# KieDani/UpliftingTableTennis

Measured on NVIDIA B200. Metric: frames_per_sec_detect_decode, higher is better.
Workload: dtype tf32

## Files before the change

### upliftingtabletennis_b200/csrc/conv_umma.cu

```cuda
#include <cuda.h>

#include <string.h>

#include <algorithm>
#include <vector>

#include "hrnet.h"
#include "umma_prims.h"

namespace {

using namespace umma;

constexpr int BW = 128;
constexpr int THREADS = 192;
constexpr int THREADS_HF = 320;

constexpr int pow2_cols(int c) { return c <= 32 ? 32 : c <= 64 ? 64 : c <= 128 ? 128 : c <= 256 ? 256 : 512; }
constexpr int al1024(int b) { return (b + 1023) & ~1023; }

template <int KS, int S, int CIN, int COUT, int R, int STAGES, int RB, int KCO = 0, int ESZ = 2, int HF = 0>
struct Cfg {
  static constexpr int KCMAX = 128 / ESZ;
  static constexpr int KC = KCO ? KCO : (CIN < KCMAX ? CIN : KCMAX);
  static constexpr int NKC = CIN / KC;
  static constexpr int ROWB = KC * ESZ;
  static constexpr int KSTEPS = ROWB / 32;
  static constexpr int PAD = KS / 2;
  static constexpr bool FUSE = KS == 3 && S == 1 && 3 * COUT <= 256;
  static constexpr int NPY = S == 2 ? 2 : 1;
  static constexpr int NBOX = S == 2 ? 2 : 1;
  static constexpr int TW = S == 2 ? BW + 1 : (HF ? BW : BW + 2 * PAD);
  static constexpr int OUTW = HF ? BW - 2 : BW;
  static constexpr int TR = S == 2 ? R + 1 : R + 2 * PAD;
  static constexpr int BOX_BYTES = TR * TW * ROWB;
  static constexpr int BOX_AL = al1024(BOX_BYTES);
  static constexpr int STAGE_BYTES = NBOX * BOX_AL;
// ... 19 lines not shown
  static constexpr uint32_t SWZ = ROWB == 32 ? 1u : ROWB == 64 ? 3u : 7u;
  static_assert(S == 1 || KS == 3, "stride 2 is implemented for 3x3 only");
  static_assert(!HF || (KS == 3 && S == 1 && 9 * COUT <= 256 && COUT == 16 && !RB), "horizontal tap fusion: 3x3 stride 1, 16 output channels, no staged residual");
  static_assert(2 * ACC_COLS <= 512, "accumulators exceed TMEM");
  static constexpr bool PIPE = S == 1 && !RB && !HF && ACC_COLS >= 64 && (ESZ == 4 || COUT >= 64);
  static constexpr int GMAX = (ESZ == 2 && !PIPE) ? 64 : 32;
  static constexpr int GCOLS = ACC_COLS < GMAX ? ACC_COLS : GMAX;
  static_assert(ESZ == 2 || ESZ == 4, "bf16 or tf32-in-fp32 elements");
  static_assert(ACC_COLS % GCOLS == 0, "the epilogue drains whole groups of accumulator columns");
  static_assert(ROWB == 32 || ROWB == 64 || ROWB == 128, "a K-chunk is one 32/64/128-byte swizzled row");
  static_assert(COUT % 16 == 0 && COUT <= 256 && CIN % 16 == 0, "bad channel counts");
  static_assert(SMEM_BYTES <= 232448, "shared memory budget");
};

struct KMaps {
  CUtensorMap m[4];
  CUtensorMap res;
};

struct KArgs {
  const void* w;
  const float* bias;
  void* out;
  const void* res[3];
  int rsh[3];
  int nres;
  int res_tma;
  int dual;
  int n, h, w_img, cout_total;
  int relu;
  int tiles_x, tiles_y, total;
};

template <int KS, int S, int CIN, int COUT, int R, int STAGES, int RB, int KCO = 0, int ESZ = 2, int HF = 0>
__global__ void __launch_bounds__(HF ? THREADS_HF : THREADS, 1) conv_umma_kernel(const __grid_constant__ KMaps maps, const KArgs a) {
  constexpr int NTHR = HF ? THREADS_HF : THREADS;
  using C = Cfg<KS, S, CIN, COUT, R, STAGES, RB, KCO, ESZ, HF>;
  extern __shared__ uint8_t smem_raw[];
  uint8_t* smem = reinterpret_cast<uint8_t*>((reinterpret_cast<uintptr_t>(smem_raw) + 1023) & ~(uintptr_t)1023);
  uint8_t* sW = smem;
  uint8_t* sA = smem + C::W_BYTES_AL;
  uint8_t* sR = sA + STAGES * C::STAGE_BYTES;
  float* sBias = reinterpret_cast<float*>(sR + C::RES_BYTES);
  float* sXch = sBias + COUT;
  uint64_t* bars = reinterpret_cast<uint64_t*>(sXch + C::XCH_BYTES / 4);
  uint32_t* tmem_slot = reinterpret_cast<uint32_t*>(bars + 2 * STAGES + 6);
  uint8_t* sStage = reinterpret_cast<uint8_t*>((reinterpret_cast<uintptr_t>(bars) + 256 + 127) & ~(uintptr_t)127);
  const uint32_t bar_full = smem_u32(bars), bar_empty = bar_full + 8 * STAGES, bar_tfull = bar_empty + 8 * STAGES,
                 bar_tempty = bar_tfull + 16, bar_rfull = bar_tempty + 16;
  const int tid = threadIdx.x, warp = tid >> 5, lane = tid & 31;
  const int n_off = blockIdx.y * COUT;
  const bool res_tma = RB && a.res_tma;

  {
    const uint4* wsrc = reinterpret_cast<const uint4*>(a.w) + (size_t)blockIdx.y * (C::W_BYTES / 16);
    const uint32_t wbase = smem_u32(sW);
    constexpr int CPR = C::ROWB / 16;
    for (int i = tid; i < C::W_BYTES / 16; i += NTHR) {
      uint32_t addr = wbase + (i / CPR) * C::ROWB + (i % CPR) * 16;
      addr ^= ((addr >> 7) & C::SWZ) << 4;
      *reinterpret_cast<uint4*>(sW + (addr - wbase)) = __ldg(wsrc + i);
    }
    for (int i = tid; i < COUT; i += NTHR) sBias[i] = a.bias[n_off + i];
  }
  if (tid == 0) {
    for (int s = 0; s < STAGES; ++s) {
      mbar_init(bar_full + 8 * s, 1);
      mbar_init(bar_empty + 8 * s, 1);
    }
    for (int i = 0; i < 2; ++i) {
// ... 131 lines not shown
    const int q = warp & 3;
    const int m = q * 32 + lane;
    constexpr int GCOLS = C::GCOLS;
    constexpr int NSUB = GCOLS / 16;
    constexpr int RW = 4 * ESZ;
    const uint32_t lane_base = tmem + ((uint32_t)(q * 32) << 16);
    const int eg = (warp - 2) >> 2;
    if (eg == 0)
      for (int c = 0; c < 2 * C::ACC_COLS; c += 16) tmem_zero16(lane_base + c);
    tmem_wait_st();
    fence_before();
    __syncwarp();
    if (lane == 0) {
      mbar_arrive(bar_tempty);
      mbar_arrive(bar_tempty + 8);
    }
    auto add_words = [](float* f, const uint32_t* w) {
      if (ESZ == 2) {
#pragma unroll
        for (int j = 0; j < 8; ++j) {
          f[2 * j] += __uint_as_float(w[j] << 16);
          f[2 * j + 1] += __uint_as_float(w[j] & 0xffff0000u);
        }
      } else {
#pragma unroll
        for (int j = 0; j < 16; ++j) f[j] += __uint_as_float(w[j]);
      }
    };
    uint32_t tcount = 0;
    for (int tile = blockIdx.x; tile < a.total; tile += gridDim.x, ++tcount) {
      const int tx = tile % a.tiles_x, ty = (tile / a.tiles_x) % a.tiles_y, img = tile / (a.tiles_x * a.tiles_y);
      const uint32_t acc = tcount & 1, aph = (tcount >> 1) & 1;
      const int ox = HF ? tx * C::OUTW + m - 1 : tx * BW + m;
      if (res_tma) mbar_wait(bar_rfull + 8 * acc, aph);
      mbar_wait(bar_tfull + 8 * acc, aph);
      fence_after();
      if constexpr (HF != 0) {
        const uint32_t tbase = lane_base + acc * C::ACC_COLS;
        float* xme = sXch + (q * 2) * R * COUT;
#pragma unroll 1
        for (int r = eg; r < R; r += 2) {
          uint32_t e0[16], e2[16];
          tmem_ld16(tbase + (R - 1 - r) * 3 * COUT, e0);
          tmem_ld16(tbase + (R - 1 - r) * 3 * COUT + 2 * COUT, e2);
          tmem_wait_ld();
          if (lane == 31) {
#pragma unroll
            for (int j = 0; j < 16; ++j) xme[r * COUT + j] = __uint_as_float(e0[j]);
          }
          if (lane == 0) {
#pragma unroll
            for (int j = 0; j < 16; ++j) xme[R * COUT + r * COUT + j] = __uint_as_float(e2[j]);
          }
        }
        asm volatile("bar.sync 1, 256;" ::: "memory");
        const float* xprev = sXch + ((q > 0 ? q - 1 : 0) * 2) * R * COUT;
        const float* xnext = sXch + ((q < 3 ? q + 1 : 3) * 2 + 1) * R * COUT;
#pragma unroll 1
        for (int r = eg; r < R; r += 2) {
          uint32_t v0[16], v1[16], v2[16];
          const uint32_t ta = tbase + (R - 1 - r) * 3 * COUT;
          tmem_ld16(ta, v0);
          tmem_ld16(ta + COUT, v1);
          tmem_ld16(ta + 2 * COUT, v2);
          tmem_wait_ld();
          tmem_zero16(ta);
// ... 122 lines not shown
            if (!(ox < a.w_img && oy < a.h)) continue;
            float f[16];
#pragma unroll
            for (int j = 0; j < 16; ++j) f[j] = __uint_as_float(v[g & 1][sb][j]) + sBias[c0 + j];
            if (nres > 0) add_words(f, rv[g & 1][sb]);
            if (a.relu) {
#pragma unroll
              for (int j = 0; j < 16; ++j) f[j] = fmaxf(f[j], 0.f);
            }
            char* op = (char*)a.out + ((((size_t)img * a.h + oy) * a.w_img + ox) * a.cout_total + n_off + c0) * ESZ;
            if (ESZ == 2) {
              uint32_t o[8];
#pragma unroll
              for (int j = 0; j < 8; ++j) {
                __nv_bfloat162 b2 = __floats2bfloat162_rn(f[2 * j], f[2 * j + 1]);
                o[j] = *reinterpret_cast<uint32_t*>(&b2);
              }
              stg256(op, o);
            } else {
              uint32_t o[16];
#pragma unroll
              for (int j = 0; j < 16; ++j) o[j] = __float_as_uint(f[j]);
              stg256(op, o);
              stg256(op + 32, o + 8);
            }
          }
          if (g + 1 < G) {
            tmem_wait_ld();
#pragma unroll
            for (int sb = 0; sb < NSUB; ++sb) tmem_zero16(tbase + (g + 1) * GCOLS + sb * 16);
          }
        }
      } else {
#pragma unroll 1
      for (int g0 = 0; g0 < C::ACC_COLS; g0 += GCOLS) {
        uint32_t v[NSUB][16];
        const uint32_t taddr = lane_base + acc * C::ACC_COLS + g0;
#pragma unroll
        for (int sb = 0; sb < NSUB; ++sb) tmem_ld16(taddr + sb * 16, v[sb]);
        uint32_t rv[NSUB][RW], rx[NSUB][2][RW];
        const int nres = a.nres;
#pragma unroll
        for (int sb = 0; sb < NSUB; ++sb) {
          const int col = g0 + sb * 16, r = R - 1 - col / COUT, c0 = col % COUT;
          const int oy = ty * R + r;
          const bool live = ox < a.w_img && oy < a.h;
#pragma unroll
          for (int j = 0; j < RW; ++j) rv[sb][j] = 0;
          if (nres > 0) {
            if (res_tma) {
              const uint32_t row = smem_u32(sR + (acc * C::NRB + c0 / C::CB) * C::RBOX_BYTES) + (r * BW + m) * C::RROWB;
              const uint32_t swz = ((row >> 7) & C::RSWZ) << 4;
#pragma unroll
              for (int i = 0; i < RW / 4; ++i) lds128((row + (c0 % C::CB) * ESZ + 16 * i) ^ swz, &rv[sb][4 * i]);
            } else if (live) {
              const int sh = a.rsh[0];
              const char* rp = (const char*)a.res[0] +
                               ((((size_t)img * (a.h >> sh) + (oy >> sh)) * (a.w_img >> sh) + (ox >> sh)) * a.cout_total + n_off + c0) * ESZ;
#pragma unroll
              for (int i = 0; i < RW / 8; ++i) ldg256(rp + 32 * i, &rv[sb][8 * i]);
            }
#pragma unroll
            for (int rr = 1; rr < 3; ++rr) {
              if (rr < nres && live) {
                const int sh = a.rsh[rr];
                const char* rp = (const char*)a.res[rr] +
                                 ((((size_t)img * (a.h >> sh) + (oy >> sh)) * (a.w_img >> sh) + (ox >> sh)) * a.cout_total + n_off + c0) * ESZ;
#pragma unroll
                for (int i = 0; i < RW / 8; ++i) ldg256(rp + 32 * i, &rx[sb][rr - 1][8 * i]);
              }
            }
          }
        }
        tmem_wait_ld();
#pragma unroll
        for (int sb = 0; sb < NSUB; ++sb) tmem_zero16(taddr + sb * 16);
#pragma unroll
        for (int sb = 0; sb < NSUB; ++sb) {
          const int col = g0 + sb * 16, r = R - 1 - col / COUT, c0 = col % COUT;
          const int oy = ty * R + r;
          if (!(ox < a.w_img && oy < a.h)) continue;
          float f[16];
#pragma unroll
          for (int j = 0; j < 16; ++j) f[j] = __uint_as_float(v[sb][j]) + sBias[c0 + j];
          if (nres > 0) {
            add_words(f, rv[sb]);
#pragma unroll
            for (int rr = 1; rr < 3; ++rr) {
              if (rr >= nres) break;
              add_words(f, rx[sb][rr - 1]);
            }
          }
          if (a.relu) {
#pragma unroll
            for (int j = 0; j < 16; ++j) f[j] = fmaxf(f[j], 0.f);
          }
          char* op = (char*)a.out + ((((size_t)img * a.h + oy) * a.w_img + ox) * a.cout_total + n_off + c0) * ESZ;
          if (ESZ == 2) {
            uint32_t o[8];
#pragma unroll
            for (int j = 0; j < 8; ++j) {
              __nv_bfloat162 b2 = __floats2bfloat162_rn(f[2 * j], f[2 * j + 1]);
              o[j] = *reinterpret_cast<uint32_t*>(&b2);
            }
            stg256(op, o);
          } else {
            uint32_t o[16];
#pragma unroll
            for (int j = 0; j < 16; ++j) o[j] = __float_as_uint(f[j]);
            stg256(op, o);
            stg256(op + 32, o + 8);
          }
        }
      }
      }
      tmem_wait_st();
      fence_before();
      __syncwarp();
      if (lane == 0) mbar_arrive(bar_tempty + 8 * acc);
    }
  }
  fence_before();
  __syncthreads();
  if (warp == 2) tmem_dealloc(tmem, C::TMEM_COLS);
}

int cout_tile(const TtkConv& cv, int esz) { return (cv.k == 3 && cv.cout_p == 128 && cv.cin_p >= 64) ? (esz == 2 ? 64 : 32) : cv.cout_p; }
bool fused_ky(const TtkConv& cv, int esz) { return cv.k == 3 && cv.stride == 1 && 3 * cout_tile(cv, esz) <= 256; }
bool fused_h(const TtkConv& cv, int esz) { return esz == 4 && cv.k == 3 && cv.stride == 1 && cv.cin_p == 128 && cv.cout_p == 16; }
int kc_of(const TtkConv& cv, int esz) {
  if (esz == 2) {
    if (cv.k == 3 && cv.stride == 1 && cv.cin_p >= 64) return 32;
    if (cv.k == 3 && cv.stride == 2 && cv.cin_p >= 64) return 32;
    return cv.cin_p < 64 ? cv.cin_p : 64;
  }
  if (cv.k == 3 && cv.stride == 1 && cv.cin_p == 128 && cv.cout_p == 16) return 16;
  if (cv.k == 3 && cv.cin_p >= 64) return 8;
  if (cv.k == 3 && cv.stride == 2 && cv.cin_p == 32 && cv.cout_p == 128) return 8;
  if (cv.k == 3) return 16;
  return 32;
}

CUtensorMapSwizzle swizzle_for(int row_bytes) {
  return row_bytes == 32 ? CU_TENSOR_MAP_SWIZZLE_32B : row_bytes == 64 ? CU_TENSOR_MAP_SWIZZLE_64B : CU_TENSOR_MAP_SWIZZLE_128B;
}

float round_tf32(float v) {
  uint32_t u;
  memcpy(&u, &v, 4);
  u += 0xfffu + ((u >> 13) & 1u);
  u &= ~0x1fffu;
  memcpy(&v, &u, 4);
  return v;
}

template <int KS, int S, int CIN, int COUT, int R, int STAGES, int RB, int KCO = 0, int ESZ = 2, int HF = 0>
int launch(const TtkConv& cv, const ConvLaunch& a, cudaStream_t st) {
  using C = Cfg<KS, S, CIN, COUT, R, STAGES, RB, KCO, ESZ, HF>;
  if (C::KC != kc_of(cv, ESZ) || COUT != cout_tile(cv, ESZ) || (HF != 0) != fused_h(cv, ESZ)) {
    ttk_set_error("conv %s: kernel K-chunk %d / output slice %d differ from the packed weights' %d / %d", cv.name.c_str(), C::KC, COUT,
                  kc_of(cv, ESZ), cout_tile(cv, ESZ));
    return TTK_ERR_STATE;
  }
  EncodeFn encode = get_encode();
  if (!encode) {
    ttk_set_error("cuTensorMapEncodeTiled is not available from the driver");
    return TTK_ERR_CUDA;
  }
  static TtkPerDevice attr;
  if (attr.first()) {
    TTK_CUDA(cudaFuncSetAttribute(conv_umma_kernel<KS, S, CIN, COUT, R, STAGES, RB, KCO, ESZ, HF>, cudaFuncAttributeMaxDynamicSharedMemorySize,
                                  C::SMEM_BYTES));
  }
  if (S == 2 && ((a.hin & 1) || (a.win & 1))) return TTK_ERR_UNSUPPORTED;
  const CUtensorMapDataType in_type = ESZ == 2 ? CU_TENSOR_MAP_DATA_TYPE_BFLOAT16 : CU_TENSOR_MAP_DATA_TYPE_TFLOAT32;
  const CUtensorMapDataType res_type = ESZ == 2 ? CU_TENSOR_MAP_DATA_TYPE_BFLOAT16 : CU_TENSOR_MAP_DATA_TYPE_FLOAT32;
  KMaps maps;
  cuuint32_t box[4] = {(cuuint32_t)C::KC, (cuuint32_t)C::TW, (cuuint32_t)C::TR, 1};
  cuuint32_t es[4] = {1, 1, 1, 1};
  for (int i = 0; i < (S == 2 ? 4 : 1); ++i) {
    const int py = i >> 1, px = i & 1;
    cuuint64_t dims[4] = {(cuuint64_t)CIN, (cuuint64_t)(a.win / S), (cuuint64_t)(a.hin / S), (cuuint64_t)a.n};
    cuuint64_t strides[3] = {(cuuint64_t)CIN * ESZ * S, (cuuint64_t)a.win * CIN * ESZ * S, (cuuint64_t)a.hin * a.win * CIN * ESZ};
    void* base = (char*)const_cast<void*>(a.in) + ((size_t)py * a.win + px) * CIN * ESZ;
    const CUresult r = encode(&maps.m[i], in_type, 4, base, dims, strides, box, es, CU_TENSOR_MAP_INTERLEAVE_NONE, swizzle_for(C::ROWB),
                              CU_TENSOR_MAP_L2_PROMOTION_L2_256B, CU_TENSOR_MAP_FLOAT_OOB_FILL_NONE);
    if (r != CUDA_SUCCESS) {
      ttk_set_error("cuTensorMapEncodeTiled failed (%d) for conv %s", (int)r, cv.name.c_str());
      return TTK_ERR_CUDA;
    }
  }
  for (int i = (S == 2 ? 4 : 1); i < 4; ++i) maps.m[i] = maps.m[0];
  const bool res_tma = RB && a.nres > 0 && a.res_shift[0] == 0;
  maps.res = maps.m[0];
  if (res_tma) {
    cuuint64_t dims[4] = {(cuuint64_t)a.cout, (cuuint64_t)a.wout, (cuuint64_t)a.hout, (cuuint64_t)a.n};
    cuuint64_t strides[3] = {(cuuint64_t)a.cout * ESZ, (cuuint64_t)a.wout * a.cout * ESZ, (cuuint64_t)a.hout * a.wout * a.cout * ESZ};
    cuuint32_t rbox[4] = {(cuuint32_t)C::CB, (cuuint32_t)BW, (cuuint32_t)R, 1};
    const CUresult r = encode(&maps.res, res_type, 4, const_cast<void*>(a.res[0]), dims, strides, rbox, es, CU_TENSOR_MAP_INTERLEAVE_NONE,
                              swizzle_for(C::RROWB), CU_TENSOR_MAP_L2_PROMOTION_L2_256B, CU_TENSOR_MAP_FLOAT_OOB_FILL_NONE);
    if (r != CUDA_SUCCESS) {
      ttk_set_error("cuTensorMapEncodeTiled (residual) failed (%d) for conv %s", (int)r, cv.name.c_str());
      return TTK_ERR_CUDA;
    }
  }
  KArgs k;
  k.w = ESZ == 2 ? (const void*)cv.w_umma : (const void*)cv.w_umma32;
  k.bias = cv.bias;
  k.out = a.out;
  for (int i = 0; i < 3; ++i) {
    k.res[i] = a.res[i];
    k.rsh[i] = a.res_shift[i];
  }
  k.nres = a.nres;
  k.res_tma = res_tma ? 1 : 0;
  k.dual = 0;
  k.n = a.n;
  k.h = a.hout;
  k.w_img = a.wout;
  k.cout_total = a.cout;
  k.relu = a.relu;
  k.tiles_x = ttk_cdiv(a.wout, C::OUTW);
  k.tiles_y = ttk_cdiv(a.hout, R);
  k.total = k.tiles_x * k.tiles_y * a.n;
  const int nsplit = a.cout / COUT;
  int occ = std::min(232448 / (C::SMEM_BYTES + 1024), 512 / C::TMEM_COLS);
  occ = std::max(1, std::min(occ, 2));
  const int gx = std::max(1, std::min(k.total, ttk_num_sms() * occ / nsplit));
  dim3 grid(gx, nsplit);
  conv_umma_kernel<KS, S, CIN, COUT, R, STAGES, RB, KCO, ESZ, HF><<<grid, HF ? THREADS_HF : THREADS, C::SMEM_BYTES, st>>>(maps, k);
  TTK_LAUNCH_CHECK();
  return TTK_OK;
}

template <int ESZ>
int launch_dual(const void* w_dual, const float* bias_dual, const ConvLaunch& a, cudaStream_t st) {
  constexpr int R = 2, STAGES = 3, KC = 128 / ESZ, CINK = ESZ == 2 ? 128 : 96;
  using C = Cfg<1, 1, CINK, 128, R, STAGES, 0, 0, ESZ>;
  EncodeFn encode = get_encode();
  if (!encode) return TTK_ERR_UNSUPPORTED;
  static TtkPerDevice attr;
  if (attr.first()) {
    TTK_CUDA(cudaFuncSetAttribute(conv_umma_kernel<1, 1, CINK, 128, R, STAGES, 0, 0, ESZ>, cudaFuncAttributeMaxDynamicSharedMemorySize, C::SMEM_BYTES));
  }
  KMaps maps;
  cuuint32_t box[4] = {(cuuint32_t)KC, (cuuint32_t)BW, (cuuint32_t)R, 1};
  cuuint32_t es[4] = {1, 1, 1, 1};
  const void* ins[2] = {a.in, a.in2};
  const int cins[2] = {a.cin, a.cin2};
  for (int i = 0; i < 2; ++i) {
    cuuint64_t dims[4] = {(cuuint64_t)cins[i], (cuuint64_t)a.win, (cuuint64_t)a.hin, (cuuint64_t)a.n};
    cuuint64_t strides[3] = {(cuuint64_t)cins[i] * ESZ, (cuuint64_t)a.win * cins[i] * ESZ, (cuuint64_t)a.hin * a.win * cins[i] * ESZ};
    const CUresult r = encode(&maps.m[i], ESZ == 2 ? CU_TENSOR_MAP_DATA_TYPE_BFLOAT16 : CU_TENSOR_MAP_DATA_TYPE_TFLOAT32, 4, const_cast<void*>(ins[i]),
                              dims, strides, box, es, CU_TENSOR_MAP_INTERLEAVE_NONE, CU_TENSOR_MAP_SWIZZLE_128B, CU_TENSOR_MAP_L2_PROMOTION_L2_256B,
                              CU_TENSOR_MAP_FLOAT_OOB_FILL_NONE);
    if (r != CUDA_SUCCESS) return TTK_ERR_UNSUPPORTED;
  }
  maps.m[2] = maps.m[3] = maps.res = maps.m[0];
  KArgs k;
  k.w = w_dual;
  k.bias = bias_dual;
  k.out = a.out;
  for (int i = 0; i < 3; ++i) {
// ... 46 lines not shown
    const int ct = cout_tile(cv, esz);
    const bool fused = fused_ky(cv, esz);
    const size_t count = (size_t)kk * cv.cin_p * cv.cout_p;
    std::vector<uint8_t> w(count * esz, 0);
    for (int co = 0; co < cv.cout; ++co)
      for (int ci = 0; ci < cv.cin; ++ci)
        for (int t = 0; t < kk; ++t) {
          const int kc = ci / KC, c = ci % KC, sl = co / ct, cl = co % ct;
          size_t row;
          if (fused_h(cv, esz)) {
            const int ky = t / 3, kx = t % 3;
            row = (((size_t)sl * nkc + kc) * 3 + ky) * 3 + kx;
          } else if (fused) {
            const int ky = t / 3, kx = t % 3;
            row = (((size_t)sl * nkc + kc) * 3 + kx) * 3 + ky;
          } else {
            row = ((size_t)sl * kk + t) * nkc + kc;
          }
          const float v = w_host[((size_t)co * cv.cin + ci) * kk + t];
          const size_t i = (row * ct + cl) * KC + c;
          if (esz == 2) reinterpret_cast<__nv_bfloat16*>(w.data())[i] = __float2bfloat16_rn(v);
          else reinterpret_cast<float*>(w.data())[i] = round_tf32(v);
        }
    void** dst = esz == 2 ? (void**)&cv.w_umma : (void**)&cv.w_umma32;
    if (!*dst) TTK_CUDA(cudaMalloc(dst, w.size()));
    TTK_CUDA(cudaMemcpy(*dst, w.data(), w.size(), cudaMemcpyHostToDevice));
  }
  return TTK_OK;
}

int ttk_conv_umma_launch(const TtkConv& cv, const ConvLaunch& a, cudaStream_t st, int esz) {
  const int ci = cv.cin_p, co = cout_tile(cv, esz);
  const int k = cv.k, s = cv.stride;
  if (esz == 2) {
#define TTK_UMMA(KS_, S_, CI_, CO_, R_, ST_, RB_) \
  if (k == KS_ && s == S_ && ci == CI_ && co == CO_) return launch<KS_, S_, CI_, CO_, R_, ST_, RB_>(cv, a, st);
    TTK_UMMA(3, 1, 16, 64, 4, 3, 0)
    if (k == 3 && s == 1 && ci == 64 && co == 64) return launch<3, 1, 64, 64, 4, 3, 0, 32>(cv, a, st);
    if (k == 3 && s == 1 && ci == 32 && co == 32 && a.nres == 0) return launch<3, 1, 32, 32, 8, 2, 0>(cv, a, st);
    TTK_UMMA(3, 1, 32, 32, 4, 2, 1)
    TTK_UMMA(3, 1, 16, 16, 8, 3, 1)
    if (k == 3 && s == 1 && ci == 128 && co == 16) return launch<3, 1, 128, 16, 8, 2, 0, 32>(cv, a, st);
    if (k == 3 && s == 1 && ci == 128 && co == 64) return launch<3, 1, 128, 64, 2, 2, 0, 32>(cv, a, st);
    if (k == 3 && s == 2 && ci == 128 && co == 32) return launch<3, 2, 128, 32, 2, 3, 0, 32>(cv, a, st);
    TTK_UMMA(3, 2, 16, 16, 4, 3, 0)
    TTK_UMMA(3, 2, 16, 32, 4, 3, 0)
    TTK_UMMA(3, 2, 16, 64, 4, 3, 0)
    TTK_UMMA(3, 2, 16, 128, 2, 3, 0)
    TTK_UMMA(3, 2, 32, 32, 4, 2, 0)
    TTK_UMMA(3, 2, 32, 64, 4, 2, 0)
    TTK_UMMA(3, 2, 32, 128, 2, 2, 0)
    if (k == 3 && s == 2 && ci == 64 && co == 64) return launch<3, 2, 64, 64, 2, 3, 0, 32>(cv, a, st);
    TTK_UMMA(1, 1, 64, 32, 4, 2, 0)
    TTK_UMMA(1, 1, 32, 128, 2, 3, 1)
    TTK_UMMA(1, 1, 64, 128, 2, 3, 0)
    TTK_UMMA(1, 1, 32, 16, 4, 3, 0)
    TTK_UMMA(1, 1, 64, 16, 4, 3, 0)
    TTK_UMMA(1, 1, 128, 16, 4, 2, 0)
    TTK_UMMA(1, 1, 128, 32, 4, 2, 0)
    TTK_UMMA(1, 1, 128, 64, 2, 2, 0)
#undef TTK_UMMA
    return TTK_ERR_UNSUPPORTED;
  }
#define TTK_UMMA32(KS_, S_, CI_, CO_, R_, ST_, RB_, KC_) \
  if (k == KS_ && s == S_ && ci == CI_ && co == CO_) return launch<KS_, S_, CI_, CO_, R_, ST_, RB_, KC_, 4>(cv, a, st);
  TTK_UMMA32(3, 1, 16, 64, 4, 3, 0, 16)
// ... 28 lines not shown
```

### upliftingtabletennis_b200/csrc/hrnet.cu

```cuda
#include <algorithm>
#include <map>

#include "hrnet.h"

namespace {

const int kBranchCh[4] = {16, 32, 64, 128};

int pad16(int c) { return (c + 15) / 16 * 16; }

struct Builder {
  ttk_hrnet* h;
  std::map<std::string, int> by_name;

  void add_conv(const std::string& name, const std::string& bn, int cin, int cout, int k, int stride) {
    TtkConv c;
    c.name = "model." + name;
    c.bn = bn.empty() ? "" : "model." + bn;
    c.cin = cin;
    c.cout = cout;
    c.k = k;
    c.stride = stride;
    c.cin_p = pad16(cin);
    c.cout_p = pad16(cout);
    by_name[name] = (int)h->convs.size();
    h->convs.push_back(c);
  }

  int tensor(int c, int shift) {
    TtkTensor t;
    t.c = c;
    t.shift = shift;
    t.first = -1;
    t.last = -1;
    t.offset = 0;
    h->tensors.push_back(t);
    return (int)h->tensors.size() - 1;
  }

  int conv(const std::string& name, int in, bool relu, std::vector<int> res = {}) {
    const int ci = by_name.at(name);
    const TtkConv& c = h->convs[ci];
    const TtkTensor& ti = h->tensors[in];
    const int out = tensor(c.cout_p, ti.shift + (c.stride == 2 ? 1 : 0));
    TtkOp op;
    op.type = OP_CONV;
    op.conv = ci;
    op.in = in;
    op.out = out;
    op.relu = relu;
    op.nres = (int)res.size();
    for (int i = 0; i < op.nres; ++i) op.res[i] = res[i];
    h->ops.push_back(op);
    return out;
  }

  int sum(int in, std::vector<int> res, bool relu) {
    const TtkTensor ti = h->tensors[in];
    const int out = tensor(ti.c, ti.shift);
    TtkOp op;
    op.type = OP_SUM;
    op.in = in;
    op.out = out;
    op.relu = relu;
    op.nres = (int)res.size();
    for (int i = 0; i < op.nres; ++i) op.res[i] = res[i];
    h->ops.push_back(op);
// ... 42 lines not shown
            B.add_conv(p + fmt(".%d.0", k), p + fmt(".%d.1", k), kBranchCh[j], cout, 3, 2);
          }
        }
      }
    pre.assign(kBranchCh, kBranchCh + nb);
  }
  B.add_conv("final_layers.0", "", 16, out_ch, 1, 1);
}

void build_ops(Builder& B) {
  ttk_hrnet* h = B.h;
  h->input_tensor = B.tensor(16, 0);
  int x = B.conv("conv1", h->input_tensor, true);
  x = B.conv("conv2", x, true);
  int a = B.conv("layer1.0.conv1", x, true);
  a = B.conv("layer1.0.conv2", a, true);
  const int sc = B.conv("layer1.0.downsample.0", x, false);
  x = B.conv("layer1.0.conv3", a, true, {sc});
  std::vector<int> ys = {x};
  std::vector<int> pre = {128};
  for (int stage = 2; stage <= 4; ++stage) {
    const int nb = stage;
    std::vector<int> xs;
    for (int i = 0; i < nb; ++i) {
      if (i < (int)pre.size()) {
        if (kBranchCh[i] != pre[i])
          xs.push_back(B.conv(fmt("transition%d.%d.0", stage - 1, i), ys[i], true));
        else
          xs.push_back(ys[i]);
      } else {
        xs.push_back(B.conv(fmt("transition%d.%d.0.0", stage - 1, i), ys.back(), true));
      }
    }
    for (int b = nb - 1; b >= 0; --b)
      for (int blk = 0; blk < 2; ++blk) {
        const std::string p = fmt("stage%d.0.branches.%d.%d", stage, b, blk);
        const int t = B.conv(p + ".conv1", xs[b], true);
        xs[b] = B.conv(p + ".conv2", t, true, {xs[b]});
      }
    std::vector<int> out(nb);
    for (int i = 0; i < nb; ++i) {
      std::vector<int> others;
      for (int j = 0; j < nb; ++j) {
        const std::string p = fmt("stage%d.0.fuse_layers.%d.%d", stage, i, j);
        if (j == i) {
          if (i == 0) continue;
          others.push_back(xs[j]);
        } else if (j > i) {
          others.push_back(B.conv(p + ".0", xs[j], false));
        } else if (j < i - 1) {
          int t = xs[j];
          for (int k = 0; k < i - j; ++k) t = B.conv(p + fmt(".%d.0", k), t, k != i - j - 1);
          others.push_back(t);
        }
      }
      if (i == 0) {
        out[0] = B.sum(xs[0], others, true);
      } else {
        const std::string p = fmt("stage%d.0.fuse_layers.%d.%d", stage, i, i - 1);
        out[i] = B.conv(p + ".0.0", xs[i - 1], true, others);
      }
    }
    ys = out;
    pre.assign(kBranchCh, kBranchCh + nb);
  }
  TtkOp fin;
  fin.type = OP_FINAL;
  fin.in = ys[0];
  fin.conv = B.by_name.at("final_layers.0");
  h->ops.push_back(fin);
  {
    std::vector<char> live_t(h->tensors.size(), 0), keep(h->ops.size(), 0);
    live_t[fin.in] = 1;
    keep.back() = 1;
    for (int o = (int)h->ops.size() - 2; o >= 0; --o) {
      const TtkOp& op = h->ops[o];
      if (op.out < 0 || !live_t[op.out]) continue;
      keep[o] = 1;
      live_t[op.in] = 1;
      for (int i = 0; i < op.nres; ++i) live_t[op.res[i]] = 1;
    }
    std::vector<TtkOp> kept;
    for (size_t o = 0; o < h->ops.size(); ++o)
      if (keep[o]) kept.push_back(h->ops[o]);
    h->dead_ops = (int)(h->ops.size() - kept.size());
    h->ops.swap(kept);
  }
  for (int o = 0; o + 1 < (int)h->ops.size(); ++o) {
    const TtkOp& ds = h->ops[o];
    const TtkOp& c3 = h->ops[o + 1];
    if (ds.type == OP_CONV && c3.type == OP_CONV && ds.conv == B.by_name.at("layer1.0.downsample.0") &&
        c3.conv == B.by_name.at("layer1.0.conv3") && c3.nres == 1 && c3.res[0] == ds.out) {
      h->dual_ds_op = o;
      h->dual_c3_op = o + 1;
    }
  }
  for (int o = 0; o < (int)h->ops.size(); ++o) {
    const TtkOp& op = h->ops[o];
    auto touch = [&](int t) {
      if (t < 0) return;
      if (h->tensors[t].first < 0) h->tensors[t].first = o;
      h->tensors[t].last = o;
    };
    touch(op.in);
    for (int i = 0; i < op.nres; ++i) touch(op.res[i]);
    touch(op.out);
  }
}

size_t plan_memory(ttk_hrnet* h, int bs, int H, int W, size_t elem) {
  struct Block {
    size_t off, size;
    int last;
  };
  std::vector<Block> live;
  size_t peak = 0;
  for (int o = 0; o < (int)h->ops.size(); ++o) {
    live.erase(std::remove_if(live.begin(), live.end(), [&](const Block& b) { return b.last < o; }), live.end());
    const int t = h->ops[o].out;
    if (t < 0) continue;
    TtkTensor& tt = h->tensors[t];
    size_t size = (size_t)bs * (H >> tt.shift) * (W >> tt.shift) * tt.c * elem;
    size = (size + 1023) & ~(size_t)1023;
    std::sort(live.begin(), live.end(), [](const Block& a, const Block& b) { return a.off < b.off; });
    size_t off = 0;
    for (const Block& b : live) {
      if (off + size <= b.off) break;
      off = std::max(off, b.off + b.size);
    }
    tt.offset = off;
    live.push_back({off, size, tt.last});
    peak = std::max(peak, off + size);
  }
  return peak;
}

template <typename T>
struct Io;
template <>
struct Io<float> {
  static __device__ __forceinline__ void load4(const float* p, float* v) {
    const float4 q = *reinterpret_cast<const float4*>(p);
    v[0] = q.x; v[1] = q.y; v[2] = q.z; v[3] = q.w;
  }
  static __device__ __forceinline__ void store4(float* p, const float* v) {
    *reinterpret_cast<float4*>(p) = make_float4(v[0], v[1], v[2], v[3]);
  }
};
template <>
struct Io<__nv_bfloat16> {
  static __device__ __forceinline__ void load4(const __nv_bfloat16* p, float* v) {
    const uint2 q = *reinterpret_cast<const uint2*>(p);
    const __nv_bfloat162 a = *reinterpret_cast<const __nv_bfloat162*>(&q.x);
    const __nv_bfloat162 b = *reinterpret_cast<const __nv_bfloat162*>(&q.y);
    v[0] = __low2float(a); v[1] = __high2float(a); v[2] = __low2float(b); v[3] = __high2float(b);
  }
  static __device__ __forceinline__ void store4(__nv_bfloat16* p, const float* v) {
    __nv_bfloat162 a = __floats2bfloat162_rn(v[0], v[1]);
    __nv_bfloat162 b = __floats2bfloat162_rn(v[2], v[3]);
    uint2 q;
    q.x = *reinterpret_cast<uint32_t*>(&a);
    q.y = *reinterpret_cast<uint32_t*>(&b);
    *reinterpret_cast<uint2*>(p) = q;
  }
// ... 236 lines not shown
    cudaEvent_t e;
    TTK_CUDA(cudaEventCreate(&e));
    h->events.push_back(e);
  }
  TTK_CUDA(cudaEventRecord(h->events[i], st));
  const TtkOp& op = h->ops[oi];
  ttk_hrnet::Rec r;
  r.op = oi;
  r.n = bs;
  auto numel = [&](int t) { const TtkTensor& tt = h->tensors[t]; return (double)bs * (H >> tt.shift) * (W >> tt.shift) * tt.c; };
  if (op.type == OP_CONV) {
    const TtkConv& c = h->convs[op.conv];
    const TtkTensor& to = h->tensors[op.out];
    const double opix = (double)bs * (H >> to.shift) * (W >> to.shift);
    r.flops = 2.0 * opix * c.cin * c.cout * c.k * c.k;
    r.bytes = (numel(op.in) + numel(op.out)) * elem + (double)c.cin_p * c.cout_p * c.k * c.k * elem;
    for (int k = 0; k < op.nres; ++k) r.bytes += numel(op.res[k]) * elem;
    if (h->cur_esz && h->dual_ready && h->use_dual && oi == h->dual_c3_op) {
      const TtkOp& ds = h->ops[h->dual_ds_op];
      const TtkConv& dc = h->convs[ds.conv];
      r.flops += 2.0 * opix * dc.cin * dc.cout;
      r.bytes += numel(ds.in) * elem + (double)dc.cin_p * dc.cout_p * elem - numel(op.res[0]) * elem;
    }
  } else if (op.type == OP_SUM) {
    r.flops = numel(op.out) * op.nres;
    r.bytes = (numel(op.in) + numel(op.out)) * elem;
    for (int k = 0; k < op.nres; ++k) r.bytes += numel(op.res[k]) * elem;
  } else {
    r.flops = 2.0 * bs * H * W * 16 * h->out_count;
    r.bytes = numel(op.in) * elem + (double)bs * H * W * h->out_count * 4;
  }
  h->recs.push_back(r);
  return TTK_OK;
}

int prepare_dual(ttk_hrnet* h) {
  if (h->dual_ds_op < 0) return TTK_OK;
  const TtkConv& ds = h->convs[h->ops[h->dual_ds_op].conv];
  const TtkConv& c3 = h->convs[h->ops[h->dual_c3_op].conv];
  if (ds.w_host.empty() || c3.w_host.empty()) return TTK_OK;
  std::vector<float> b(128);
  for (int co = 0; co < 128; ++co) b[co] = c3.b_host[co] + ds.b_host[co];
  for (int esz = 2; esz <= 4; esz += 2) {
    std::vector<uint8_t> w;
    ttk_conv_umma_pack_dual(c3.w_host.data(), ds.w_host.data(), esz, w);
    void** dst = esz == 2 ? &h->w_dual : &h->w_dual32;
    if (!*dst) TTK_CUDA(cudaMalloc(dst, w.size()));
    TTK_CUDA(cudaMemcpy(*dst, w.data(), w.size(), cudaMemcpyHostToDevice));
  }
  if (!h->bias_dual) TTK_CUDA(cudaMalloc((void**)&h->bias_dual, 128 * sizeof(float)));
  TTK_CUDA(cudaMemcpy(h->bias_dual, b.data(), 128 * sizeof(float), cudaMemcpyHostToDevice));
  h->dual_ready = true;
  return TTK_OK;
}

bool is_basic_block(const ttk_hrnet* h, size_t oi) {
  if (oi + 1 >= h->ops.size()) return false;
  const TtkOp &a = h->ops[oi], &b = h->ops[oi + 1];
  if (a.type != OP_CONV || b.type != OP_CONV || a.nres != 0 || !a.relu || !b.relu || b.in != a.out || b.nres != 1 || b.res[0] != a.in) return false;
  const TtkConv &c1 = h->convs[a.conv], &c2 = h->convs[b.conv];
  if (c1.k != 3 || c2.k != 3 || c1.stride != 1 || c2.stride != 1) return false;
  if (c1.cin_p != c1.cout_p || c2.cin_p != c1.cin_p || c2.cout_p != c1.cin_p) return false;
  if (c1.cin_p != 16 && c1.cin_p != 32) return false;
  if (h->tensors[a.out].last != (int)oi + 1) return false;
  return true;
}
// ... 57 lines not shown
      a.win = W >> ti.shift;
      a.hout = H >> to.shift;
      a.wout = W >> to.shift;
      a.cin = cv.cin_p;
      a.cout = cv.cout_p;
      a.relu = op.relu ? 1 : 0;
      int rc = TTK_ERR_UNSUPPORTED;
      if (dual_skipped && (int)oi == h->dual_c3_op) {
        const TtkOp& ds = h->ops[h->dual_ds_op];
        ConvLaunch d = a;
        d.nres = 0;
        d.in2 = ptr(ds.in);
        d.cin2 = h->convs[ds.conv].cin_p;
        rc = ttk_conv_umma_launch_dual(esz == 2 ? h->w_dual : h->w_dual32, h->bias_dual, d, st, esz);
        if (rc == TTK_ERR_UNSUPPORTED) {
          h->use_dual = 0;
          ConvLaunch s0;
          const TtkConv& dcv = h->convs[ds.conv];
          const TtkTensor& dti = h->tensors[ds.in];
          const TtkTensor& dto = h->tensors[ds.out];
          s0.in = ptr(ds.in);
          s0.out = ptr(ds.out);
          s0.nres = 0;
          for (int r = 0; r < 3; ++r) { s0.res[r] = nullptr; s0.res_shift[r] = 0; }
          s0.n = bs; s0.hin = H >> dti.shift; s0.win = W >> dti.shift; s0.hout = H >> dto.shift; s0.wout = W >> dto.shift;
          s0.cin = dcv.cin_p; s0.cout = dcv.cout_p; s0.relu = 0;
          rc = ttk_conv_umma_launch(dcv, s0, st, esz);
          if (rc == TTK_ERR_UNSUPPORTED) rc = launch_conv_simt<T>(dcv, s0, sizeof(T) == 2, st);
          if (rc != TTK_OK) return rc;
          h->launches++;
          rc = ttk_conv_umma_launch(cv, a, st, esz);
        }
      } else if (umma) {
        rc = ttk_conv_umma_launch(cv, a, st, esz);
      }
      if (rc == TTK_ERR_UNSUPPORTED) rc = launch_conv_simt<T>(cv, a, sizeof(T) == 2, st);
      if (rc != TTK_OK) return rc;
      h->launches++;
    } else if (op.type == OP_SUM) {
      const TtkTensor& to = h->tensors[op.out];
      const int hh = H >> to.shift, ww = W >> to.shift;
      const int cv = to.c / (32 / (int)sizeof(T));
      int cv_shift = 0;
      while ((1 << cv_shift) < cv) ++cv_shift;
      if ((1 << cv_shift) != cv || bs > 65535 || hh > 65535) {
        ttk_set_error("fuse sum: %d channels / batch %d / height %d not supported", to.c, bs, hh);
        return TTK_ERR_UNSUPPORTED;
      }
      const dim3 blocks(ttk_cdiv(ww << cv_shift, 512), hh, bs);
      int sh[3] = {0, 0, 0};
      const void* rp[3] = {nullptr, nullptr, nullptr};
      for (int r = 0; r < op.nres; ++r) {
        rp[r] = ptr(op.res[r]);
        sh[r] = h->tensors[op.res[r]].shift - to.shift;
      }
      sum_kernel<T><<<blocks, 256, 0, st>>>((const T*)ptr(op.in), (T*)ptr(op.out), (const T*)rp[0], (const T*)rp[1],
                                           (const T*)rp[2], sh[0], sh[1], sh[2], op.nres, hh, ww, to.c, cv_shift, op.relu ? 1 : 0);
      TTK_LAUNCH_CHECK();
      h->launches++;
    } else {
      const long long total = (long long)bs * H * W;
      const int blocks = (int)std::min<long long>((total + 255) / 256, (long long)ttk_num_sms() * 16);
      final_kernel<T><<<blocks, 256, h->out_count * 17 * sizeof(float), st>>>((const T*)ptr(op.in), heat, h->final_w, h->final_b,
                                                                            bs, H * W, h->out_count);
      TTK_LAUNCH_CHECK();
      h->launches++;
// ... 54 lines not shown
  delete h;
}

extern "C" int ttk_hrnet_num_convs(const ttk_hrnet* h) { return h ? (int)h->convs.size() : 0; }

extern "C" int ttk_hrnet_conv_info(const ttk_hrnet* h, int i, char* name, char* bn, int* cin, int* cout, int* k, int* stride) {
  TTK_CHECK_ARG(h && i >= 0 && i < (int)h->convs.size(), "ttk_hrnet_conv_info: bad index %d", i);
  const TtkConv& c = h->convs[i];
  if (name) snprintf(name, 128, "%s", c.name.c_str());
  if (bn) snprintf(bn, 128, "%s", c.bn.c_str());
  if (cin) *cin = c.cin;
  if (cout) *cout = c.cout;
  if (k) *k = c.k;
  if (stride) *stride = c.stride;
  return TTK_OK;
}

extern "C" int ttk_hrnet_set_conv(ttk_hrnet* h, int i, const float* w_host, const float* b_host) {
  TTK_CHECK_ARG(h && i >= 0 && i < (int)h->convs.size(), "ttk_hrnet_set_conv: bad index %d", i);
  TTK_CHECK_ARG(w_host && b_host, "ttk_hrnet_set_conv: null pointer");
  if (int rc = ttk_bind_device(&h->device, "ttk_hrnet_set_conv")) return rc;
  TtkConv& c = h->convs[i];
  const int kk = c.k * c.k;
  if (i == (int)h->convs.size() - 1) {
    std::vector<float> w((size_t)h->out_count * 16, 0.f), b(h->out_count);
    for (int o = 0; o < h->out_count; ++o) {
      for (int ci = 0; ci < c.cin; ++ci) w[o * 16 + ci] = w_host[(size_t)(h->out_first + o) * c.cin + ci];
      b[o] = b_host[h->out_first + o];
    }
    int rc = upload(&h->final_w, w);
    if (rc) return rc;
    rc = upload(&h->final_b, b);
    if (rc) return rc;
    c.set = true;
    return TTK_OK;
  }
  std::vector<float> w((size_t)kk * c.cin_p * c.cout_p, 0.f), wr(w.size(), 0.f), b(c.cout_p, 0.f);
  for (int co = 0; co < c.cout; ++co) {
    b[co] = b_host[co];
    for (int ci = 0; ci < c.cin; ++ci)
      for (int t = 0; t < kk; ++t) {
        const float v = w_host[((size_t)co * c.cin + ci) * kk + t];
        w[((size_t)t * c.cin_p + ci) * c.cout_p + co] = v;
        wr[((size_t)t * c.cin_p + ci) * c.cout_p + co] = bf16_round(v);
      }
  }
  c.w_host.assign(w_host, w_host + (size_t)c.cout * c.cin * kk);
  c.b_host.assign(b_host, b_host + c.cout);
  h->dual_ready = false;
  int rc = upload(&c.w_f32, w);
  if (rc) return rc;
  rc = upload(&c.w_bfr, wr);
  if (rc) return rc;
  rc = upload(&c.bias, b);
  if (rc) return rc;
  rc = ttk_conv_umma_pack(c, w_host);
  if (rc) return rc;
  c.set = true;
  return TTK_OK;
}

extern "C" size_t ttk_hrnet_workspace_bytes(const ttk_hrnet* h, int batch, int height, int width, int dtype) {
  if (!h || batch <= 0 || height <= 0 || width <= 0) return 0;
  const int bs = std::min(batch, h->subbatch);
  return plan_memory(const_cast<ttk_hrnet*>(h), bs, height, width, dtype == TTK_BF16 ? 2 : 4);
}
// ... 119 lines not shown
```

### upliftingtabletennis_b200/csrc/hrnet.h

```cpp
#pragma once
#include <stdint.h>

#include <string>
#include <vector>

#include "ttk_internal.h"

struct TtkConv {
  std::string name, bn;
  int cin, cout, k, stride;
  int cin_p, cout_p;
  bool set = false;
  float* w_f32 = nullptr;
  float* w_bfr = nullptr;
  float* bias = nullptr;
  __nv_bfloat16* w_umma = nullptr;
  float* w_umma32 = nullptr;
  std::vector<float> w_host, b_host;
};

struct TtkTensor {
  int c;
  int shift;
  int first, last;
  size_t offset;
};

enum { OP_CONV = 0, OP_SUM = 1, OP_FINAL = 2 };

struct TtkOp {
  int type;
  int conv = -1;
  int in = -1, out = -1;
  int nres = 0;
  int res[3] = {-1, -1, -1};
  bool relu = false;
};

struct ConvLaunch {
  const void* in;
  void* out;
  const void* res[3];
  int res_shift[3];
  int nres;
  int n, hin, win, hout, wout;
  int cin, cout;
  int relu;
  const void* in2 = nullptr;
  int cin2 = 0;
};

struct ttk_hrnet {
  int in_ch, out_ch, out_first, out_count;
  int device = -1;
  std::vector<TtkConv> convs;
  std::vector<TtkTensor> tensors;
  std::vector<TtkOp> ops;
  int input_tensor = -1;
  int dead_ops = 0;
  int subbatch = 16;
  int launches = 0;
  int force_simt = 0;
  float* final_w = nullptr;
  float* final_b = nullptr;
  int dual_ds_op = -1, dual_c3_op = -1;
  void* w_dual = nullptr;
  void* w_dual32 = nullptr;
  float* bias_dual = nullptr;
  bool dual_ready = false;
  int use_dual = 1;
  int cur_esz = 0;
  int use_block_fusion = 1;
  int profile = 0;
  std::vector<cudaEvent_t> events;
  struct Rec { int op; int n; double flops, bytes; };
  std::vector<Rec> recs;
};

int ttk_conv_umma_launch(const TtkConv& cv, const ConvLaunch& a, cudaStream_t st, int esz = 2);
int ttk_conv_umma_pack(TtkConv& cv, const float* w_host);
int ttk_conv_umma_launch_dual(const void* w_dual, const float* bias_dual, const ConvLaunch& a, cudaStream_t st, int esz = 2);
void ttk_conv_umma_pack_dual(const float* w3, const float* wd, int esz, std::vector<uint8_t>& out);

int ttk_block_umma_launch(const TtkConv& c1, const TtkConv& c2, const void* x, void* y, int n, int h, int w, cudaStream_t st, int esz = 2);
```

Before: 670.6.

## Fold HRNet fuse-sum and final 1x1 head into TF32 conv epilogue

Detects a conv followed by a ReLU sum of upsampled branch tensors (and optionally the final 1x1 heatmap conv), then launches a specialised TF32 16-channel UMMA conv variant. Its epilogue adds the upsampled residuals, applies ReLU, and writes either the summed tensor or the head outputs directly, with the head weights passed as kernel parameters. This removes separate sum and final-head launches and the global-memory round trips of intermediate tensors. It also reorders graph construction so the stage fuse-layer upsample convs for branch 0 run before the fold point, and extends tensor lifetimes for the memory planner. In exchange it adds register pressure from the prefetched fold residuals and a larger kernel-parameter block.

```diff
diff --git a/upliftingtabletennis_b200/csrc/conv_umma.cu b/upliftingtabletennis_b200/csrc/conv_umma.cu
--- a/upliftingtabletennis_b200/csrc/conv_umma.cu
+++ b/upliftingtabletennis_b200/csrc/conv_umma.cu
@@ -3,6 +3,7 @@
 #include <string.h>
 
 #include <algorithm>
+#include <type_traits>
 #include <vector>
 
 #include "hrnet.h"
@@ -88,10 +89,26 @@
   int tiles_x, tiles_y, total;
 };
 
-template <int KS, int S, int CIN, int COUT, int R, int STAGES, int RB, int KCO = 0, int ESZ = 2, int HF = 0>
-__global__ void __launch_bounds__(HF ? THREADS_HF : THREADS, 1) conv_umma_kernel(const __grid_constant__ KMaps maps, const KArgs a) {
+constexpr int HEAD_MAX = 13;
+struct KFold : KArgs {
+  const float* fres[3];
+  int fsh[3];
+  int nfold;
+  float* fout;
+  float* heat;
+  int out_count;
+  float hw[HEAD_MAX * 16];
+  float hb[HEAD_MAX];
+};
+template <int FOLD>
+using KArgsOf = std::conditional_t<FOLD != 0, KFold, KArgs>;
+
+template <int KS, int S, int CIN, int COUT, int R, int STAGES, int RB, int KCO = 0, int ESZ = 2, int HF = 0, int FOLD = 0>
+__global__ void __launch_bounds__(HF ? THREADS_HF : THREADS, 1) conv_umma_kernel(const __grid_constant__ KMaps maps, const KArgsOf<FOLD> a) {
   constexpr int NTHR = HF ? THREADS_HF : THREADS;
   using C = Cfg<KS, S, CIN, COUT, R, STAGES, RB, KCO, ESZ, HF>;
+  static_assert(FOLD == 0 || (ESZ == 4 && COUT == 16 && RB && !C::PIPE && !HF && C::GCOLS == 2 * COUT && R % 2 == 0),
+                "the fold rides on the TF32 16-channel staged-residual epilogue, two rows (2k + 1, 2k) per column group");
   extern __shared__ uint8_t smem_raw[];
   uint8_t* smem = reinterpret_cast<uint8_t*>((reinterpret_cast<uintptr_t>(smem_raw) + 1023) & ~(uintptr_t)1023);
   uint8_t* sW = smem;
@@ -289,6 +306,22 @@
       const int tx = tile % a.tiles_x, ty = (tile / a.tiles_x) % a.tiles_y, img = tile / (a.tiles_x * a.tiles_y);
       const uint32_t acc = tcount & 1, aph = (tcount >> 1) & 1;
       const int ox = HF ? tx * C::OUTW + m - 1 : tx * BW + m;
+      uint32_t fr[FOLD ? C::ACC_COLS / C::GCOLS : 1][FOLD ? 3 : 1][16];
+      if constexpr (FOLD != 0) {
+#pragma unroll
+        for (int g = 0; g < C::ACC_COLS / C::GCOLS; ++g) {
+          const int oy = ty * R + R - 1 - g * C::GCOLS / COUT;
+#pragma unroll
+          for (int t = 0; t < 3; ++t) {
+            if (t < a.nfold && ox < a.w_img && oy < a.h) {
+              const int sh = a.fsh[t];
+              const char* fp = (const char*)a.fres[t] + ((((size_t)img * (a.h >> sh) + (oy >> sh)) * (a.w_img >> sh) + (ox >> sh)) * 16) * 4;
+              ldg256(fp, &fr[g][t][0]);
+              ldg256(fp + 32, &fr[g][t][8]);
+            }
+          }
+        }
+      }
       if (res_tma) mbar_wait(bar_rfull + 8 * acc, aph);
       mbar_wait(bar_tfull + 8 * acc, aph);
       fence_after();
@@ -477,7 +510,7 @@
           }
         }
       } else {
-#pragma unroll 1
+#pragma unroll(FOLD ? C::ACC_COLS / GCOLS : 1)
       for (int g0 = 0; g0 < C::ACC_COLS; g0 += GCOLS) {
         uint32_t v[NSUB][16];
         const uint32_t taddr = lane_base + acc * C::ACC_COLS + g0;
@@ -505,6 +538,7 @@
 #pragma unroll
               for (int i = 0; i < RW / 8; ++i) ldg256(rp + 32 * i, &rv[sb][8 * i]);
             }
+            if constexpr (FOLD == 0) {
 #pragma unroll
             for (int rr = 1; rr < 3; ++rr) {
               if (rr < nres && live) {
@@ -515,6 +549,7 @@
                 for (int i = 0; i < RW / 8; ++i) ldg256(rp + 32 * i, &rx[sb][rr - 1][8 * i]);
               }
             }
+            }
           }
         }
         tmem_wait_ld();
@@ -530,18 +565,22 @@
           for (int j = 0; j < 16; ++j) f[j] = __uint_as_float(v[sb][j]) + sBias[c0 + j];
           if (nres > 0) {
             add_words(f, rv[sb]);
+            if constexpr (FOLD == 0) {
 #pragma unroll
             for (int rr = 1; rr < 3; ++rr) {
               if (rr >= nres) break;
               add_words(f, rx[sb][rr - 1]);
             }
+            }
           }
           if (a.relu) {
 #pragma unroll
             for (int j = 0; j < 16; ++j) f[j] = fmaxf(f[j], 0.f);
           }
-          char* op = (char*)a.out + ((((size_t)img * a.h + oy) * a.w_img + ox) * a.cout_total + n_off + c0) * ESZ;
-          if (ESZ == 2) {
+          const size_t po = (((size_t)img * a.h + oy) * a.w_img + ox) * a.cout_total + n_off + c0;
+          char* op = (char*)a.out + po * ESZ;
+          if (FOLD == 2) {
+          } else if (ESZ == 2) {
             uint32_t o[8];
 #pragma unroll
             for (int j = 0; j < 8; ++j) {
@@ -555,6 +594,34 @@
             for (int j = 0; j < 16; ++j) o[j] = __float_as_uint(f[j]);
             stg256(op, o);
             stg256(op + 32, o + 8);
+          }
+          if constexpr (FOLD != 0) {
+#pragma unroll
+            for (int t = 0; t < 3; ++t) {
+              if (t >= a.nfold) break;
+#pragma unroll
+              for (int j = 0; j < 16; ++j) f[j] += __uint_as_float(fr[g0 / GCOLS][t][j]);
+            }
+#pragma unroll
+            for (int j = 0; j < 16; ++j) f[j] = fmaxf(f[j], 0.f);
+            if constexpr (FOLD == 1) {
+              uint32_t o[16];
+#pragma unroll
+              for (int j = 0; j < 16; ++j) o[j] = __float_as_uint(f[j]);
+              stg256((char*)a.fout + po * 4, o);
+              stg256((char*)a.fout + po * 4 + 32, o + 8);
+            } else {
+              const size_t plane = (size_t)a.h * a.w_img;
+              float* hp = a.heat + ((size_t)img * a.out_count * a.h + oy) * a.w_img + ox;
+#pragma unroll
+              for (int o = 0; o < HEAD_MAX; ++o) {
+                if (o >= a.out_count) break;
+                float acc = 0.f;
+#pragma unroll
+                for (int c = 0; c < 16; ++c) acc = fmaf(f[c], a.hw[o * 16 + c], acc);
+                hp[o * plane] = acc + a.hb[o];
+              }
+            }
           }
         }
       }
@@ -599,7 +666,7 @@
   return v;
 }
 
-template <int KS, int S, int CIN, int COUT, int R, int STAGES, int RB, int KCO = 0, int ESZ = 2, int HF = 0>
+template <int KS, int S, int CIN, int COUT, int R, int STAGES, int RB, int KCO = 0, int ESZ = 2, int HF = 0, int FOLD = 0>
 int launch(const TtkConv& cv, const ConvLaunch& a, cudaStream_t st) {
   using C = Cfg<KS, S, CIN, COUT, R, STAGES, RB, KCO, ESZ, HF>;
   if (C::KC != kc_of(cv, ESZ) || COUT != cout_tile(cv, ESZ) || (HF != 0) != fused_h(cv, ESZ)) {
@@ -614,7 +681,7 @@
   }
   static TtkPerDevice attr;
   if (attr.first()) {
-    TTK_CUDA(cudaFuncSetAttribute(conv_umma_kernel<KS, S, CIN, COUT, R, STAGES, RB, KCO, ESZ, HF>, cudaFuncAttributeMaxDynamicSharedMemorySize,
+    TTK_CUDA(cudaFuncSetAttribute(conv_umma_kernel<KS, S, CIN, COUT, R, STAGES, RB, KCO, ESZ, HF, FOLD>, cudaFuncAttributeMaxDynamicSharedMemorySize,
                                   C::SMEM_BYTES));
   }
   if (S == 2 && ((a.hin & 1) || (a.win & 1))) return TTK_ERR_UNSUPPORTED;
@@ -649,7 +716,7 @@
       return TTK_ERR_CUDA;
     }
   }
-  KArgs k;
+  KArgsOf<FOLD> k;
   k.w = ESZ == 2 ? (const void*)cv.w_umma : (const void*)cv.w_umma32;
   k.bias = cv.bias;
   k.out = a.out;
@@ -668,12 +735,28 @@
   k.tiles_x = ttk_cdiv(a.wout, C::OUTW);
   k.tiles_y = ttk_cdiv(a.hout, R);
   k.total = k.tiles_x * k.tiles_y * a.n;
+  if constexpr (FOLD != 0) {
+    for (int i = 0; i < 3; ++i) {
+      k.fres[i] = (const float*)a.fold_res[i];
+      k.fsh[i] = a.fold_shift[i];
+    }
+    k.nfold = a.nfold;
+    k.fout = (float*)a.fold_out;
+    k.heat = a.heat;
+    k.out_count = FOLD == 2 ? a.out_count : 0;
+    memset(k.hw, 0, sizeof(k.hw));
+    memset(k.hb, 0, sizeof(k.hb));
+    if (FOLD == 2) {
+      memcpy(k.hw, a.head_w, (size_t)a.out_count * 16 * sizeof(float));
+      memcpy(k.hb, a.head_b, (size_t)a.out_count * sizeof(float));
+    }
+  }
   const int nsplit = a.cout / COUT;
   int occ = std::min(232448 / (C::SMEM_BYTES + 1024), 512 / C::TMEM_COLS);
   occ = std::max(1, std::min(occ, 2));
   const int gx = std::max(1, std::min(k.total, ttk_num_sms() * occ / nsplit));
   dim3 grid(gx, nsplit);
-  conv_umma_kernel<KS, S, CIN, COUT, R, STAGES, RB, KCO, ESZ, HF><<<grid, HF ? THREADS_HF : THREADS, C::SMEM_BYTES, st>>>(maps, k);
+  conv_umma_kernel<KS, S, CIN, COUT, R, STAGES, RB, KCO, ESZ, HF, FOLD><<<grid, HF ? THREADS_HF : THREADS, C::SMEM_BYTES, st>>>(maps, k);
   TTK_LAUNCH_CHECK();
   return TTK_OK;
 }
@@ -786,6 +869,14 @@
 int ttk_conv_umma_launch(const TtkConv& cv, const ConvLaunch& a, cudaStream_t st, int esz) {
   const int ci = cv.cin_p, co = cout_tile(cv, esz);
   const int k = cv.k, s = cv.stride;
+  if (a.nfold) {
+    if (esz != 4 || k != 3 || s != 1 || ci != 16 || co != 16 || a.nres != 1 || a.res_shift[0] != 0 || !a.relu || a.nfold > 3 ||
+        (a.hout & 1) || (a.heat ? a.out_count < 1 || a.out_count > HEAD_MAX : !a.fold_out))
+      return TTK_ERR_UNSUPPORTED;
+    for (int i = 0; i < a.nfold; ++i)
+      if (a.fold_shift[i] < 1) return TTK_ERR_UNSUPPORTED;
+    return a.heat ? launch<3, 1, 16, 16, 4, 3, 1, 16, 4, 0, 2>(cv, a, st) : launch<3, 1, 16, 16, 4, 3, 1, 16, 4, 0, 1>(cv, a, st);
+  }
   if (esz == 2) {
 #define TTK_UMMA(KS_, S_, CI_, CO_, R_, ST_, RB_) \
   if (k == KS_ && s == S_ && ci == CI_ && co == CO_) return launch<KS_, S_, CI_, CO_, R_, ST_, RB_>(cv, a, st);
diff --git a/upliftingtabletennis_b200/csrc/hrnet.cu b/upliftingtabletennis_b200/csrc/hrnet.cu
--- a/upliftingtabletennis_b200/csrc/hrnet.cu
+++ b/upliftingtabletennis_b200/csrc/hrnet.cu
@@ -33,6 +33,7 @@
     t.shift = shift;
     t.first = -1;
     t.last = -1;
+    t.last_mem = -1;
     t.offset = 0;
     h->tensors.push_back(t);
     return (int)h->tensors.size() - 1;
@@ -141,12 +142,15 @@
         xs.push_back(B.conv(fmt("transition%d.%d.0.0", stage - 1, i), ys.back(), true));
       }
     }
-    for (int b = nb - 1; b >= 0; --b)
+    std::vector<int> up0(nb, -1);
+    for (int b = nb - 1; b >= 0; --b) {
       for (int blk = 0; blk < 2; ++blk) {
         const std::string p = fmt("stage%d.0.branches.%d.%d", stage, b, blk);
         const int t = B.conv(p + ".conv1", xs[b], true);
         xs[b] = B.conv(p + ".conv2", t, true, {xs[b]});
       }
+      if (b > 0) up0[b] = B.conv(fmt("stage%d.0.fuse_layers.0.%d.0", stage, b), xs[b], false);
+    }
     std::vector<int> out(nb);
     for (int i = 0; i < nb; ++i) {
       std::vector<int> others;
@@ -156,7 +160,7 @@
           if (i == 0) continue;
           others.push_back(xs[j]);
         } else if (j > i) {
-          others.push_back(B.conv(p + ".0", xs[j], false));
+          others.push_back(i == 0 ? up0[j] : B.conv(p + ".0", xs[j], false));
         } else if (j < i - 1) {
           int t = xs[j];
           for (int k = 0; k < i - j; ++k) t = B.conv(p + fmt(".%d.0", k), t, k != i - j - 1);
@@ -214,6 +218,21 @@
     touch(op.in);
     for (int i = 0; i < op.nres; ++i) touch(op.res[i]);
     touch(op.out);
+  }
+  for (int o = 0; o + 1 < (int)h->ops.size(); ++o) {
+    const TtkOp &c2 = h->ops[o], &sm = h->ops[o + 1];
+    if (c2.type != OP_CONV || sm.type != OP_SUM || sm.in != c2.out || !sm.relu || sm.nres < 1 || sm.nres > 3) continue;
+    TtkFold f{o, o + 1, -1};
+    if (o + 2 < (int)h->ops.size() && h->ops[o + 2].type == OP_FINAL && h->ops[o + 2].in == sm.out && h->tensors[c2.out].last == o + 1 &&
+        h->tensors[sm.out].last == o + 2)
+      f.final_op = o + 2;
+    h->folds.push_back(f);
+  }
+  for (TtkTensor& t : h->tensors) t.last_mem = t.last;
+  for (const TtkFold& f : h->folds) {
+    const TtkOp& c2 = h->ops[f.conv_op];
+    h->tensors[c2.in].last_mem = std::max(h->tensors[c2.in].last, f.sum_op);
+    for (int i = 0; i < c2.nres; ++i) h->tensors[c2.res[i]].last_mem = std::max(h->tensors[c2.res[i]].last, f.sum_op);
   }
 }
 
@@ -238,7 +257,7 @@
       off = std::max(off, b.off + b.size);
     }
     tt.offset = off;
-    live.push_back({off, size, tt.last});
+    live.push_back({off, size, tt.last_mem});
     peak = std::max(peak, off + size);
   }
   return peak;
@@ -541,6 +560,20 @@
   }
   h->recs.push_back(r);
   return TTK_OK;
+}
+
+void profile_fold(ttk_hrnet* h, const TtkFold& f, int bs, int H, int W, size_t elem) {
+  ttk_hrnet::Rec& r = h->recs.back();
+  auto numel = [&](int t) { const TtkTensor& tt = h->tensors[t]; return (double)bs * (H >> tt.shift) * (W >> tt.shift) * tt.c; };
+  const TtkOp &c2 = h->ops[f.conv_op], &sm = h->ops[f.sum_op];
+  r.flops += numel(sm.out) * sm.nres;
+  for (int k = 0; k < sm.nres; ++k) r.bytes += numel(sm.res[k]) * elem;
+  if (f.final_op < 0) {
+    r.bytes += numel(sm.out) * elem;
+  } else {
+    r.flops += 2.0 * bs * H * W * 16 * h->out_count;
+    r.bytes += (double)bs * H * W * h->out_count * 4 - numel(c2.out) * elem;
+  }
 }
 
 int prepare_dual(ttk_hrnet* h) {
@@ -664,6 +697,36 @@
           rc = ttk_conv_umma_launch(cv, a, st, esz);
         }
       } else if (umma) {
+        const TtkFold* fold = nullptr;
+        if (esz == 4 && h->use_block_fusion == 1)
+          for (const TtkFold& f : h->folds)
+            if (f.conv_op == (int)oi) fold = &f;
+        if (fold && fold->final_op >= 0 && h->final_w_host.empty()) fold = nullptr;
+        if (fold) {
+          const TtkOp& sm = h->ops[fold->sum_op];
+          ConvLaunch fa = a;
+          fa.nfold = sm.nres;
+          for (int r = 0; r < sm.nres; ++r) {
+            fa.fold_res[r] = ptr(sm.res[r]);
+            fa.fold_shift[r] = h->tensors[sm.res[r]].shift - to.shift;
+          }
+          if (fold->final_op >= 0) {
+            fa.heat = heat;
+            fa.head_w = h->final_w_host.data();
+            fa.head_b = h->final_b_host.data();
+            fa.out_count = h->out_count;
+          } else {
+            fa.fold_out = ptr(sm.out);
+          }
+          rc = ttk_conv_umma_launch(cv, fa, st, esz);
+          if (rc == TTK_OK) {
+            if (h->profile) profile_fold(h, *fold, bs, H, W, sizeof(T));
+            h->launches++;
+            oi = fold->final_op >= 0 ? fold->final_op : fold->sum_op;
+            continue;
+          }
+          if (rc != TTK_ERR_UNSUPPORTED) return rc;
+        }
         rc = ttk_conv_umma_launch(cv, a, st, esz);
       }
       if (rc == TTK_ERR_UNSUPPORTED) rc = launch_conv_simt<T>(cv, a, sizeof(T) == 2, st);
@@ -784,6 +847,8 @@
     if (rc) return rc;
     rc = upload(&h->final_b, b);
     if (rc) return rc;
+    h->final_w_host = w;
+    h->final_b_host = b;
     c.set = true;
     return TTK_OK;
   }
diff --git a/upliftingtabletennis_b200/csrc/hrnet.h b/upliftingtabletennis_b200/csrc/hrnet.h
--- a/upliftingtabletennis_b200/csrc/hrnet.h
+++ b/upliftingtabletennis_b200/csrc/hrnet.h
@@ -23,6 +23,7 @@
   int c;
   int shift;
   int first, last;
+  int last_mem;
   size_t offset;
 };
 
@@ -48,6 +49,18 @@
   int relu;
   const void* in2 = nullptr;
   int cin2 = 0;
+  int nfold = 0;
+  const void* fold_res[3] = {nullptr, nullptr, nullptr};
+  int fold_shift[3] = {0, 0, 0};
+  void* fold_out = nullptr;
+  float* heat = nullptr;
+  const float* head_w = nullptr;
+  const float* head_b = nullptr;
+  int out_count = 0;
+};
+
+struct TtkFold {
+  int conv_op, sum_op, final_op;
 };
 
 struct ttk_hrnet {
@@ -63,12 +76,14 @@
   int force_simt = 0;
   float* final_w = nullptr;
   float* final_b = nullptr;
+  std::vector<float> final_w_host, final_b_host;
   int dual_ds_op = -1, dual_c3_op = -1;
   void* w_dual = nullptr;
   void* w_dual32 = nullptr;
   float* bias_dual = nullptr;
   bool dual_ready = false;
   int use_dual = 1;
+  std::vector<TtkFold> folds;
   int cur_esz = 0;
   int use_block_fusion = 1;
   int profile = 0;
```

New measurement: 696.1 (median of 6 runs). 1.04x the previous value.
